# lab-oak/oak

Measured on AMD Instinct MI355X. Metric: turn-steps/s (batched playouts), higher is better.
Workload: dtype u16

## Files before the change

include/oakgpu.h:

```cpp
#ifndef OAKGPU_H
#define OAKGPU_H
#include <stddef.h>
#include <stdint.h>

#ifdef __cplusplus
extern "C" {
#endif

#define OAKGPU_BATTLE_SIZE 384
#define OAKGPU_DURATIONS_SIZE 8
#define OAKGPU_ACTIONS_SIZE 16
#define OAKGPU_MAX_CHOICES 9
#define OAKGPU_TEAMS_SIZE 60

typedef struct oakgpu_ctx oakgpu_ctx;
typedef struct oakgpu_net oakgpu_net;

int oakgpu_create(oakgpu_ctx **out, int device);
void oakgpu_destroy(oakgpu_ctx *ctx);
const char *oakgpu_last_error(void);
int oakgpu_set_stream(oakgpu_ctx *ctx, void *hip_stream);
void *oakgpu_get_stream(oakgpu_ctx *ctx);
int oakgpu_synchronize(oakgpu_ctx *ctx);
int oakgpu_set_kernel_timing(oakgpu_ctx *ctx, int on);
int oakgpu_get_leaf_kernel_ms(oakgpu_ctx *ctx, float ms[3]);
int oakgpu_set_playouts_per_lane(oakgpu_ctx *ctx, int k);
int oakgpu_set_regroup(oakgpu_ctx *ctx, int rounds, int suspend_below, int shrink);
int oakgpu_set_tail_pack(oakgpu_ctx *ctx, int below, int waves, int lanes);
int oakgpu_set_queue_order(oakgpu_ctx *ctx, int on);
int oakgpu_set_spread(oakgpu_ctx *ctx, int lanes);
int oakgpu_set_migration(oakgpu_ctx *ctx, int mode, int long_steps, int adopters);
int oakgpu_set_migration_window(oakgpu_ctx *ctx, int window);
int oakgpu_set_standstill_skip(oakgpu_ctx *ctx, int on);
#define OAKGPU_MOVE_CARRY_DEFAULT 32
int oakgpu_set_move_carry(oakgpu_ctx *ctx, int below);
#define OAKGPU_MOVE_CARRY_DRY_DEFAULT 0
int oakgpu_set_move_carry_dry(oakgpu_ctx *ctx, int below);
#define OAKGPU_LEAN_ROLLOUT_DEFAULT 1
int oakgpu_set_lean_rollout(oakgpu_ctx *ctx, int on);
int oakgpu_last_launch_lean(oakgpu_ctx *ctx);
#define OAKGPU_CTL_FAST_FORWARDED 44
#define OAKGPU_CTL_SKIPPED_STEPS 45
int oakgpu_get_queue_counters(oakgpu_ctx *ctx, uint32_t *out64);
int oakgpu_device_count(void);

int oakgpu_rollout_dev(oakgpu_ctx *ctx, const uint8_t *battles, const uint8_t *durations,
                       const uint8_t *results_in, uint8_t *prng_state, uint32_t n, uint32_t max_steps,
                       int prep, uint8_t *results_out, uint32_t *steps_out, float *values_out,
                       uint8_t *battles_out, uint8_t *durations_out);
int oakgpu_rollout(oakgpu_ctx *ctx, const uint8_t *battles, const uint8_t *durations,
                   const uint8_t *results_in, uint8_t *prng_state, uint32_t n, uint32_t max_steps, int prep,
                   uint8_t *results_out, uint32_t *steps_out, float *values_out, uint8_t *battles_out,
                   uint8_t *durations_out);

typedef struct {
  const uint8_t *battles, *durations, *results_in;
  uint8_t *prng_state;
  uint32_t n;
  uint8_t *results_out;
  uint32_t *steps_out;
  float *values_out;
// ... 619 lines not shown
```

oak_amd/_lib.py:

```python
import ctypes as C
import os

_HERE = os.path.dirname(os.path.abspath(__file__))
LIB_PATH = os.environ.get("OAKGPU_LIB") or os.path.join(_HERE, "liboakgpu.so")

SYMBOLS = [
    "oakgpu_create", "oakgpu_destroy", "oakgpu_last_error", "oakgpu_set_stream", "oakgpu_get_stream", "oakgpu_synchronize", "oakgpu_set_kernel_timing", "oakgpu_get_leaf_kernel_ms", "oakgpu_set_playouts_per_lane", "oakgpu_set_regroup", "oakgpu_set_tail_pack", "oakgpu_set_queue_order", "oakgpu_queue_order", "oakgpu_set_spread", "oakgpu_set_migration", "oakgpu_set_migration_window", "oakgpu_set_standstill_skip", "oakgpu_set_move_carry", "oakgpu_set_move_carry_dry", "oakgpu_set_lean_rollout", "oakgpu_last_launch_lean", "oakgpu_get_queue_counters",
    "oakgpu_device_count", "oakgpu_rollout_dev", "oakgpu_rollout", "oakgpu_rollout_group_dev", "oakgpu_rollout_group",
    "oakgpu_mt19937_fill", "oakgpu_rollout_draws_dev", "oakgpu_rollout_shared_device", "oakgpu_update_dev", "oakgpu_update",
    "oakgpu_choices_dev", "oakgpu_choices", "oakgpu_init_battles_dev", "oakgpu_init_battles",
    "oakgpu_set_ou_pools", "oakgpu_random_ou_battles_dev",
    "oakgpu_net_load", "oakgpu_net_load_memory", "oakgpu_net_free", "oakgpu_net_shape", "oakgpu_net_set_main_precision", "oakgpu_net_main_precision", "oakgpu_net_policy_form",
    "oakgpu_net_load_discrete", "oakgpu_net_load_discrete_memory", "oakgpu_net_is_discrete", "oakgpu_leaf_eval_discrete_raw_dev",
    "oakgpu_leaf_eval_dev", "oakgpu_leaf_eval", "oakgpu_leaf_eval_cached_dev", "oakgpu_leaf_cache_last_count", "oakgpu_leaf_embed_forms", "oakgpu_leaf_eval_policy_dev", "oakgpu_leaf_eval_policy",
    "oakgpu_heap_create", "oakgpu_heap_destroy", "oakgpu_heap_empty", "oakgpu_heap_clear", "oakgpu_heap_kind", "oakgpu_heap_nodes", "oakgpu_heap_update",
    "oakgpu_heap_root_stats", "oakgpu_heap_child_stats", "oakgpu_search_heap", "oakgpu_search_agent_heap", "oakgpu_heap_check_shards", "oakgpu_heap_selftest",
    "oakgpu_tree_step_dev", "oakgpu_search", "oakgpu_search_many", "oakgpu_search_agent", "oakgpu_agent_networks_clear", "oakgpu_bandit_replay", "oakgpu_bandit_select_run", "oakgpu_solve_matrix",
    "oakgpu_segment_mean_dev", "oakgpu_comm_unique_id", "oakgpu_comm_create", "oakgpu_comm_destroy", "oakgpu_all_gather_dev",
    "oakgpu_root_steps_create", "oakgpu_root_steps_destroy", "oakgpu_root_steps_launch_dev", "oakgpu_root_steps_capacity", "oakgpu_root_steps_reserve",
    "oakgpu_endless_battle_check", "oakgpu_frames_size", "oakgpu_frames_write", "oakgpu_frames_read", "oakgpu_selfplay_game", "oakgpu_selfplay_games", "oakgpu_poke_engine_eval_dev", "oakgpu_poke_engine_eval",
    "oakgpu_replay_index", "oakgpu_replay_records_dev", "oakgpu_replay_records", "oakgpu_engine_switches",
    "oakgpu_corpus_create", "oakgpu_corpus_destroy", "oakgpu_corpus_info", "oakgpu_frames_encode_dev", "oakgpu_frames_sample_dev", "oakgpu_encode_battles_dev",
    "oakgpu_frames_encode", "oakgpu_frames_sample",
    "oakgpu_corpus_frame_bases", "oakgpu_corpus_chunks", "oakgpu_corpus_states_dev", "oakgpu_corpus_states", "oakgpu_corpus_inference_dev", "oakgpu_corpus_loss_dev",
    "oakgpu_corpus_inference", "oakgpu_corpus_evaluate",
    "oakgpu_party_table_create", "oakgpu_party_table_destroy", "oakgpu_party_table_fill_dev", "oakgpu_party_table_fill", "oakgpu_leaf_eval_table_dev",
    "oakgpu_leaf_eval_policy_table_dev", "oakgpu_party_table_last_misses", "oakgpu_party_table_rows", "oakgpu_party_table_width", "oakgpu_party_key", "oakgpu_party_variant",
    "oakgpu_set_search_party_table", "oakgpu_search_party_table_stats", "oakgpu_leaf_eval_table", "oakgpu_leaf_eval_policy_table",
    "oakgpu_policy_games_dev", "oakgpu_policy_games", "oakgpu_policy_games_last_stats",
    "oakgpu_forest_create", "oakgpu_forest_destroy", "oakgpu_forest_check", "oakgpu_forest_search_dev", "oakgpu_forest_search", "oakgpu_forest_nodes",
    "oakgpu_forest_last_stats", "oakgpu_search_stream", "oakgpu_agent_params",
    "oakgpu_forest_selfplay_check", "oakgpu_forest_selfplay_dev", "oakgpu_forest_selfplay_records", "oakgpu_forest_selfplay", "oakgpu_forest_selfplay_last_stats",
    "oakgpu_selfplay_pick_host",
    "oakgpu_forest_match_check", "oakgpu_forest_match_dev", "oakgpu_forest_match", "oakgpu_forest_match_last_stats", "oakgpu_match_pick_host",
    "oakgpu_forest_match_set_records", "oakgpu_forest_match_records",
    "oakgpu_forest_create_kept", "oakgpu_forest_create_kept_check", "oakgpu_forest_kept_tree_bytes", "oakgpu_forest_advance_dev", "oakgpu_forest_advance",
    "oakgpu_forest_search_kept_dev", "oakgpu_forest_search_kept", "oakgpu_forest_keep_stats", "oakgpu_forest_mismatch", "oakgpu_forest_node_counts",
    "oakgpu_forest_selfplay_nodes_kept", "oakgpu_forest_selfplay_keep_stats",
    "oakgpu_nash_solve_dev", "oakgpu_solve_matrices", "oakgpu_nash_soft_host", "oakgpu_nash_round_host", "oakgpu_nash_width4_max_entry",
    "oakgpu_forest_selfplay_last_traffic",
# ... 192 lines not shown
    "pkmn_gen1_battle_options_chance_actions", "pkmn_gen1_battle_options_chance_durations",
    "pkmn_result_type", "pkmn_result_p1", "pkmn_result_p2",
]

_lib = None


class OakGpuError(RuntimeError):
    pass


def load():
    global _lib
    if _lib is not None:
        return _lib
    if not os.path.exists(LIB_PATH):
        raise OakGpuError("liboakgpu.so not built: run `python -c 'import __graft_entry__ as g; g.build()'` "
                          "(hipcc --offload-arch=gfx950); there is no CPU fallback")
    lib = C.CDLL(LIB_PATH)
    vp, u32, u64, i32 = C.c_void_p, C.c_uint32, C.c_uint64, C.c_int
    lib.oakgpu_create.argtypes = [C.POINTER(vp), i32]
    lib.oakgpu_destroy.argtypes = [vp]
    lib.oakgpu_destroy.restype = None
    lib.oakgpu_last_error.restype = C.c_char_p
    lib.oakgpu_set_stream.argtypes = [vp, vp]
    lib.oakgpu_get_stream.argtypes = [vp]
    lib.oakgpu_get_stream.restype = vp
    lib.oakgpu_synchronize.argtypes = [vp]
    lib.oakgpu_set_kernel_timing.argtypes = [vp, i32]
    lib.oakgpu_get_leaf_kernel_ms.argtypes = [vp, C.POINTER(C.c_float)]
    lib.oakgpu_set_playouts_per_lane.argtypes = [vp, i32]
    lib.oakgpu_set_regroup.argtypes = [vp, i32, i32, i32]
    lib.oakgpu_set_tail_pack.argtypes = [vp, i32, i32, i32]
    lib.oakgpu_set_queue_order.argtypes = [vp, i32]
    lib.oakgpu_queue_order.argtypes = [vp, C.POINTER(RolloutBatch), u32, vp, C.POINTER(u32)]
    lib.oakgpu_set_spread.argtypes = [vp, i32]
    lib.oakgpu_set_migration.argtypes = [vp, i32, i32, i32]
    lib.oakgpu_set_migration_window.argtypes = [vp, i32]
    lib.oakgpu_set_standstill_skip.argtypes = [vp, i32]
    lib.oakgpu_set_move_carry.argtypes = [vp, i32]
    lib.oakgpu_set_move_carry_dry.argtypes = [vp, i32]
    lib.oakgpu_set_lean_rollout.argtypes = [vp, i32]
    lib.oakgpu_last_launch_lean.argtypes = [vp]
    lib.oakgpu_get_queue_counters.argtypes = [vp, vp]
    lib.oakgpu_rollout_dev.argtypes = [vp, vp, vp, vp, vp, u32, u32, i32, vp, vp, vp, vp, vp]
    lib.oakgpu_rollout.argtypes = [vp, vp, vp, vp, vp, u32, u32, i32, vp, vp, vp, vp, vp]
    lib.oakgpu_rollout_group_dev.argtypes = [vp, C.POINTER(RolloutBatch), u32, u32, i32]
    lib.oakgpu_rollout_group.argtypes = [vp, C.POINTER(RolloutBatch), u32, u32, i32]
    lib.oakgpu_mt19937_fill.argtypes = [u32, u64, vp, C.c_size_t]
    lib.oakgpu_rollout_draws_dev.argtypes = [vp, vp, u32, vp, u32, vp, u32, vp, u32, vp, u32, u32, i32, vp, vp, vp, vp, vp, vp]
    lib.oakgpu_rollout_shared_device.argtypes = [vp, vp, vp, C.c_uint8, vp, u32, u32, u32, i32, vp, vp, vp, vp, vp, vp, vp]
    lib.oakgpu_poke_engine_eval_dev.argtypes = [vp, vp, u32, C.c_float, vp, vp]
    lib.oakgpu_poke_engine_eval.argtypes = [vp, vp, u32, C.c_float, vp, vp]
    lib.oakgpu_tree_step_dev.argtypes = [vp, vp, vp, vp, vp, vp, u32, u32, vp, vp, vp, vp, vp]
    lib.oakgpu_search.argtypes = [vp, vp, vp, vp, C.c_uint8, C.POINTER(SearchParams), C.POINTER(SearchOutput)]
    lib.oakgpu_heap_create.argtypes = [C.POINTER(vp)]
    lib.oakgpu_heap_destroy.argtypes = [vp]
    lib.oakgpu_heap_destroy.restype = None
    lib.oakgpu_heap_empty.argtypes = [vp]
    lib.oakgpu_heap_clear.argtypes = [vp]
    lib.oakgpu_heap_clear.restype = None
    lib.oakgpu_heap_kind.argtypes = [vp]
    lib.oakgpu_heap_nodes.argtypes = [vp]
    lib.oakgpu_heap_nodes.restype = u64
    lib.oakgpu_heap_update.argtypes = [vp, C.c_uint8, C.c_uint8, vp]
    lib.oakgpu_heap_root_stats.argtypes = [vp, i32, vp, vp, vp, vp]
# ... 227 lines not shown
```

oak_amd/csrc/oakgpu.hip:

```cpp
#include <hip/hip_runtime.h>
#include <stdint.h>
#include <stdio.h>
#include <stdlib.h>
#include <string.h>
#include <algorithm>
#include <random>
#include <mutex>
#include <string>
#include <type_traits>
#include <vector>

#include "../../include/oakgpu.h"
#include "gen1_device.hpp"
#include "gen1_regs.hpp"
#include "record_walk.hpp"
#include "oakgpu_internal.h"
#include "fast_prng.hpp"

namespace oak {
using namespace walk;

constexpr int STATE_WORDS = 96;
constexpr int TABLE_LDS_PAD = TABLE_PAD;

// ... 1343 lines not shown
  int device;
  hipStream_t stream;
  bool own_stream;
  uint8_t *d_legal, *d_pools, *d_sizes;
  int n_legal;
  int playouts_per_lane;
  uint32_t *d_queue;
  uint32_t *d_heads;
  int rounds;
  int suspend_below;
  int round_shrink;
  uint8_t *d_scratch;
  size_t scratch_n;
  int rounds_auto;
  int concurrent_hint;
  int search_party_table;
  uint64_t search_table_fills = 0, search_table_evals = 0;
  const void *ws2_owner = nullptr;
  int tail_below;
  int tail_waves;
  int tail_lanes;
  int migrate;
  int migrate_steps;
  int migrate_adopters;
  int migrate_window;
  int migrate_used;
  int spread_lanes;
  int queue_order;
  int standstill_skip;
  int move_carry;
  int move_carry_dry;
  int lean_rollout;
  int last_launch_lean;
  uint32_t *d_order;
  size_t order_n;
  uint32_t order_pair = 0;
  uint32_t ticket_epoch = 0;
  bool tickets_dirty = true;
  int n_cu;
  static constexpr int TABLE_SLOTS = 8;
  void *h_table, *d_table;
  hipEvent_t table_ev[TABLE_SLOTS];
  uint64_t table_next;
  struct Block { void *p; size_t cap; };
  std::vector<Block> stage;
  size_t stage_cursor;
  Block ws[3];
  int timing;
  hipEvent_t tev[4];
  bool tev_valid;
  Block replay_ws{nullptr, 0};
  Block games_ws{nullptr, 0};
  void *attachment = nullptr;
  void (*attachment_dtor)(void *) = nullptr;
};

static thread_local std::string g_err;
static int fail(hipError_t e, const char *what) {
  g_err = std::string(what) + ": " + hipGetErrorString(e);
  return (int)e;
}
static int bad(const char *what) {
  g_err = what;
  return -1;
}
int oakgpu_fail_hip(int e, const char *what) { return fail((hipError_t)e, what); }
int oakgpu_fail_msg(const char *what) { return bad(what); }
int oakgpu_ctx_device(const oakgpu_ctx *c) { return c->device; }
int oakgpu_ctx_enter(oakgpu_ctx *c) {
  hipError_t e = hipSetDevice(c->device);
  return e == hipSuccess ? 0 : fail(e, "hipSetDevice");
}
static void *grow_block(oakgpu_ctx *c, oakgpu_ctx::Block &b, size_t bytes) {
  if (b.cap >= bytes && b.p) return b.p;
  if (b.p) {
    (void)hipStreamSynchronize(c->stream);
    (void)hipFree(b.p);
    b.p = nullptr;
    b.cap = 0;
  }
  const size_t cap = (bytes + (1u << 20) - 1) & ~(size_t)((1u << 20) - 1);
  hipError_t e = hipMalloc(&b.p, cap);
  if (e != hipSuccess) { b.p = nullptr; fail(e, "hipMalloc(context buffer)"); return nullptr; }
  b.cap = cap;
  return b.p;
}
void **oakgpu_ctx_timing_events(oakgpu_ctx *c) { return c->timing && c->tev_valid ? (void **)c->tev : nullptr; }
void *oakgpu_ctx_workspace(oakgpu_ctx *c, int slot, size_t bytes) {
// ... 110 lines not shown
  c->timing = 0;
  c->tev_valid = false;
  c->rounds_auto = 1;
  c->concurrent_hint = 0;
  c->search_party_table = 0;
  if (const char *env = getenv("OAKGPU_PARTY_TABLE")) c->search_party_table = atoi(env) != 0;
  if (const char *env = getenv("OAKGPU_ROUNDS_AUTO")) c->rounds_auto = atoi(env) != 0;
  {
    hipDeviceProp_t prop;
    hipError_t pe = hipGetDeviceProperties(&prop, device);
    if (pe != hipSuccess) { delete c; return fail(pe, "hipGetDeviceProperties"); }
    c->n_cu = prop.multiProcessorCount > 0 ? prop.multiProcessorCount : 256;
  }
  c->rounds = 4;
  c->suspend_below = 32;
  c->round_shrink = 3;
  c->tail_below = 0;
  c->tail_waves = 0;
  if (const char *env = getenv("OAKGPU_TAIL_BELOW")) c->tail_below = atoi(env) < 0 ? 0 : atoi(env) > 64 ? 64 : atoi(env);
  if (const char *env = getenv("OAKGPU_TAIL_WAVES")) c->tail_waves = atoi(env) < 0 ? 0 : atoi(env);
  c->spread_lanes = -1;
  if (const char *env = getenv("OAKGPU_SPREAD_LANES")) c->spread_lanes = atoi(env) < -1 ? -1 : atoi(env) > 64 ? 64 : atoi(env);
  c->queue_order = 1;
  if (const char *env = getenv("OAKGPU_QUEUE_ORDER")) c->queue_order = atoi(env) != 0;
  c->standstill_skip = 1;
  if (const char *env = getenv("OAKGPU_STANDSTILL_SKIP")) c->standstill_skip = atoi(env) != 0;
  c->move_carry = OAKGPU_MOVE_CARRY_DEFAULT;
  if (const char *env = getenv("OAKGPU_MOVE_CARRY")) c->move_carry = atoi(env) < 0 ? 0 : atoi(env) > 64 ? 64 : atoi(env);
  c->move_carry_dry = OAKGPU_MOVE_CARRY_DRY_DEFAULT;
  if (const char *env = getenv("OAKGPU_MOVE_CARRY_DRY")) c->move_carry_dry = atoi(env) < 0 ? 0 : atoi(env) > 64 ? 64 : atoi(env);
  c->lean_rollout = OAKGPU_LEAN_ROLLOUT_DEFAULT;
  if (const char *env = getenv("OAKGPU_LEAN_ROLLOUT")) c->lean_rollout = atoi(env) != 0;
  c->last_launch_lean = 0;
  c->migrate = 1;
  c->migrate_steps = 300;
  c->migrate_adopters = 0;
  c->migrate_window = 48;
  c->migrate_used = 0;
  if (const char *env = getenv("OAKGPU_MIGRATE")) c->migrate = atoi(env) < 0 ? 0 : atoi(env) > 2 ? 2 : atoi(env);
  if (const char *env = getenv("OAKGPU_MIGRATE_STEPS")) c->migrate_steps = atoi(env) < 1 ? 1 : atoi(env);
  if (const char *env = getenv("OAKGPU_MIGRATE_ADOPTERS")) c->migrate_adopters = atoi(env) < 0 ? 0 : atoi(env);
  if (const char *env = getenv("OAKGPU_MIGRATE_WINDOW")) c->migrate_window = atoi(env) < 0 ? 0 : atoi(env) > 255 ? 255 : atoi(env);
  c->d_order = nullptr;
  c->order_n = 0;
  c->tail_lanes = 0;
  if (const char *env = getenv("OAKGPU_TAIL_LANES")) c->tail_lanes = atoi(env) < 0 ? 0 : atoi(env) > 64 ? 64 : atoi(env);
  if (const char *env = getenv("OAKGPU_ROUNDS")) c->rounds = atoi(env) < 1 ? 1 : atoi(env) > 8 ? 8 : atoi(env);
  if (const char *env = getenv("OAKGPU_SUSPEND_BELOW")) c->suspend_below = atoi(env) < 0 ? 0 : atoi(env) > 64 ? 64 : atoi(env);
  if (const char *env = getenv("OAKGPU_ROUND_SHRINK")) c->round_shrink = atoi(env) < 1 ? 1 : atoi(env);
  hipError_t e = hipStreamCreateWithFlags(&c->stream, hipStreamNonBlocking);
  if (e != hipSuccess) { delete c; return fail(e, "hipStreamCreate"); }
  *out = c;
  return 0;
}

void oakgpu_destroy(oakgpu_ctx *c) {
  if (!c) return;
  (void)hipSetDevice(c->device);
  (void)hipStreamSynchronize(c->stream);
  if (c->attachment && c->attachment_dtor) { c->attachment_dtor(c->attachment); c->attachment = nullptr; }
  if (c->own_stream) (void)hipStreamDestroy(c->stream);
  if (c->d_legal) (void)hipFree(c->d_legal);
  if (c->d_pools) (void)hipFree(c->d_pools);
  if (c->d_sizes) (void)hipFree(c->d_sizes);
  if (c->d_queue) (void)hipFree(c->d_queue);
  if (c->d_heads) (void)hipFree(c->d_heads);
  if (c->d_scratch) (void)hipFree(c->d_scratch);
  if (c->d_order) (void)hipFree(c->d_order);
  for (auto &b : c->stage) if (b.p) (void)hipFree(b.p);
  for (auto &b : c->ws) if (b.p) (void)hipFree(b.p);
  if (c->replay_ws.p) (void)hipFree(c->replay_ws.p);
  if (c->games_ws.p) (void)hipFree(c->games_ws.p);
  if (c->tev_valid) for (auto &e : c->tev) (void)hipEventDestroy(e);
  if (c->h_table) {
    (void)hipHostFree(c->h_table);
    (void)hipFree(c->d_table);
    for (int i = 0; i < oakgpu_ctx::TABLE_SLOTS; ++i) (void)hipEventDestroy(c->table_ev[i]);
  }
  delete c;
}

int oakgpu_set_stream(oakgpu_ctx *c, void *hip_stream) {
  if (!c) return bad("null ctx");
  if (c->own_stream) { (void)hipStreamSynchronize(c->stream); (void)hipStreamDestroy(c->stream); }
  c->stream = (hipStream_t)hip_stream;
  c->own_stream = false;
  return 0;
}

int oakgpu_set_playouts_per_lane(oakgpu_ctx *c, int k) {
// ... 65 lines not shown
  return 0;
}

int oakgpu_last_launch_lean(oakgpu_ctx *c) { return c ? c->last_launch_lean : 0; }

int oakgpu_set_search_party_table(oakgpu_ctx *c, int on) {
  if (!c) return bad("null ctx");
  const int old = c->search_party_table;
  c->search_party_table = on != 0;
  return old;
}

int oakgpu_search_party_table_stats(oakgpu_ctx *c, uint64_t *fills, uint64_t *evals) {
  if (!c) return bad("null ctx");
  if (fills) *fills = c->search_table_fills;
  if (evals) *evals = c->search_table_evals;
  return 0;
}

int oakgpu_set_queue_order(oakgpu_ctx *c, int on) {
  if (!c) return bad("null ctx");
  c->queue_order = on != 0;
  return 0;
}

int oakgpu_set_tail_pack(oakgpu_ctx *c, int below, int waves, int lanes) {
  if (!c || below < 0 || below > 64 || waves < 0 || lanes < 0 || lanes > 64) return bad("oakgpu_set_tail_pack: bad argument");
  c->tail_below = below;
  c->tail_waves = waves;
  c->tail_lanes = lanes;
  return 0;
}

void *oakgpu_get_stream(oakgpu_ctx *c) { return c ? (void *)c->stream : nullptr; }

int oakgpu_set_kernel_timing(oakgpu_ctx *c, int on) {
  if (!c) return bad("null ctx");
  HIPCHK(hipSetDevice(c->device));
  if (on && !c->tev_valid) {
    for (auto &e : c->tev) HIPCHK(hipEventCreate(&e));
    c->tev_valid = true;
  }
  c->timing = on != 0;
  return 0;
}

int oakgpu_get_leaf_kernel_ms(oakgpu_ctx *c, float ms[3]) {
  if (!c || !ms) return bad("oakgpu_get_leaf_kernel_ms: null argument");
  if (!c->timing || !c->tev_valid) return bad("oakgpu_get_leaf_kernel_ms: kernel timing is off (oakgpu_set_kernel_timing)");
  HIPCHK(hipEventSynchronize(c->tev[3]));
  for (int i = 0; i < 3; ++i) HIPCHK(hipEventElapsedTime(&ms[i], c->tev[i], c->tev[i + 1]));
  return 0;
}

int oakgpu_synchronize(oakgpu_ctx *c) {
  if (!c) return bad("null ctx");
  HIPCHK(hipStreamSynchronize(c->stream));
  if (c->d_queue && c->migrate_used) {
    uint32_t err = 0;
    HIPCHK(hipMemcpy(&err, c->d_queue + 63, 4, hipMemcpyDeviceToHost));
    c->migrate_used = 0;
    if (err) { HIPCHK(hipMemsetAsync(c->d_queue + 63, 0, 4, c->stream)); HIPCHK(hipStreamSynchronize(c->stream)); }
    if (err) return bad("rollout: a bounded wait of the long-playout migration ran out (playouts were lost) -- oakgpu_set_migration(ctx, 0, ...) turns it off");
  }
  return 0;
}
// ... 27 lines not shown
  const int slot = (int)(c->table_next++ % oakgpu_ctx::TABLE_SLOTS);
  HIPCHK(hipEventSynchronize(c->table_ev[slot]));
  oak::BatchDesc *ht = (oak::BatchDesc *)c->h_table + (size_t)slot * oak::MAX_GROUP, *dt = (oak::BatchDesc *)c->d_table + (size_t)slot * oak::MAX_GROUP;
  memcpy(ht, descs, sizeof(oak::BatchDesc) * count);
  HIPCHK(hipMemcpyAsync(dt, ht, sizeof(oak::BatchDesc) * count, hipMemcpyHostToDevice, c->stream));
  HIPCHK(hipEventRecord(c->table_ev[slot], c->stream));
  *dt_out = dt;
  return 0;
}

static int launch_queue_order(oakgpu_ctx *c, const oak::GroupArgs &g) {
  if (c->order_n < g.total) {
    if (c->d_order) { HIPCHK(hipStreamSynchronize(c->stream)); HIPCHK(hipFree(c->d_order)); c->d_order = nullptr; }
    HIPCHK(hipMalloc((void **)&c->d_order, (size_t)g.total * 4));
    c->order_n = g.total;
  }
  const uint32_t pair = 32u + 2u * c->order_pair;
  c->order_pair ^= 1u;
  hipLaunchKernelGGL(oak::k_queue_order, dim3((g.total + oak::ORDER_PER_BLOCK - 1) / oak::ORDER_PER_BLOCK), dim3(oak::ORDER_BLOCK), 0, c->stream, g, c->d_order,
                     c->d_queue, c->d_heads, pair);
  return 0;
}

static int launch_group(oakgpu_ctx *c, const oak::BatchDesc *descs, uint32_t count, uint32_t total, uint32_t max_steps, int prep) {
  HIPCHK(hipSetDevice(c->device));
  oak::BatchDesc *dt = nullptr;
  if (int r = stage_group_table(c, descs, count, &dt)) return r;
  const uint32_t n64 = (total + 63) / 64;
  uint32_t waves = (n64 + c->playouts_per_lane - 1) / c->playouts_per_lane;
  if (waves < 1) waves = 1;
  const uint32_t resident = (uint32_t)c->n_cu * 4u * 4u;
  bool saturated = waves >= resident;
  if (saturated) waves = resident;
  uint32_t spread = 0;
  if (!saturated && c->spread_lanes != 0 && !c->concurrent_hint && max_steps > 64) {
    const uint64_t slots = ((uint64_t)total + c->playouts_per_lane - 1) / c->playouts_per_lane;
    uint32_t lanes = c->spread_lanes > 0 ? (uint32_t)c->spread_lanes : (uint32_t)((slots + resident - 1) / resident);
    if (lanes < 4) lanes = 4;
    if (lanes < 64) {
      uint32_t w = (uint32_t)((slots + lanes - 1) / lanes);
      if (w > resident) w = resident;
      if (w > waves) { waves = w; spread = lanes; }
    }
  }
  const bool tail_pack = saturated && c->tail_below > 0 && max_steps > 64;
  const uint32_t adopters = (uint32_t)(c->migrate_adopters > 0 ? c->migrate_adopters : (c->n_cu + 3) / 4);
  const bool migrate = !tail_pack && max_steps > (uint32_t)c->migrate_steps && waves > adopters &&
                       (c->migrate == 2 || (c->migrate == 1 && saturated && max_steps >= 500));
  const int rounds = tail_pack ? 2 : migrate ? 1 : ((!c->rounds_auto || (c->concurrent_hint && !saturated && max_steps > 64)) && c->suspend_below > 0 && waves >= 8) ? c->rounds : 1;
  if ((rounds > 1 || migrate) && c->scratch_n < total) {
    if (c->d_scratch) { HIPCHK(hipStreamSynchronize(c->stream)); HIPCHK(hipFree(c->d_scratch)); c->d_scratch = nullptr; }
    HIPCHK(hipMalloc((void **)&c->d_scratch, (size_t)total * (384 + 8 + 4 + 4) + (((size_t)total + 15) & ~(size_t)15)));
    c->scratch_n = total;
    c->tickets_dirty = true;
  }
  const size_t lq = 24 * 64 * 4 + oak::TABLE_LDS_PAD + oak::COLD_LDS_BYTES;
  uint8_t *sb = c->d_scratch, *sd = sb ? sb + (size_t)c->scratch_n * 384 : nullptr;
  uint32_t *lists[2] = {sd ? (uint32_t *)(sd + (size_t)c->scratch_n * 8) : nullptr, nullptr};
  lists[1] = lists[0] ? lists[0] + c->scratch_n : nullptr;
  uint8_t *sres = lists[1] ? (uint8_t *)(lists[1] + c->scratch_n) : nullptr;
  const oak::GroupArgs g{dt, count, total, max_steps, prep};
  bool lean = c->lean_rollout != 0;
  for (uint32_t i = 0; i < count; ++i) lean = lean && !descs[i].durations_out;
  c->last_launch_lean = lean;
  const uint32_t *order = nullptr;
  if (c->queue_order && max_steps > 250 && total >= 8192) {
    if (int r = launch_queue_order(c, g)) return r;
    order = c->d_order;
  } else {
    hipLaunchKernelGGL(oak::k_clear_launch_words, dim3(1), dim3(256), 0, c->stream, c->d_queue, c->d_heads);
  }
  if (migrate) {
    if (++c->ticket_epoch == 0 || c->tickets_dirty) {
      HIPCHK(hipMemsetAsync(lists[0], 0, (size_t)c->scratch_n * 8, c->stream));
      if (c->ticket_epoch == 0) c->ticket_epoch = 1;
      c->tickets_dirty = false;
    }
    c->migrate_used = 1;
  } else if (rounds > 1) c->tickets_dirty = true;
  for (int r = 0; r < rounds; ++r) {
    oak::RoundArgs q{};
    q.order = r == 0 ? order : nullptr;
    q.long_steps = (uint32_t)(c->migrate_steps > 0xFFFF ? 0xFFFF : c->migrate_steps) | (uint32_t)(c->migrate_window > 0 ? c->migrate_window : 256) << 16;
    q.no_skip = c->standstill_skip ? 0u : 1u;
    q.move_carry = (uint32_t)c->move_carry;
    q.stats = c->d_queue + OAKGPU_CTL_FAST_FORWARDED;
    if (migrate) { q.adopt_ctl = c->d_queue + 40; q.adopt_list = (uint64_t *)lists[0]; q.epoch = c->ticket_epoch; q.n_adopters = adopters; }
    q.list_in = r ? lists[(r - 1) & 1] : nullptr;
    q.n_in = r ? c->d_queue + 2 * r - 1 : nullptr;
    q.list_out = lists[r & 1];
    q.count_out = c->d_queue + 2 * r + 1;
    q.sb = sb; q.sd = sd; q.sres = sres;
    q.suspend_below = r + 1 < rounds ? (uint32_t)(tail_pack ? c->tail_below : c->suspend_below) : 0u;
    q.move_carry_dry = c->move_carry_dry > 0 ? std::max((uint32_t)c->move_carry_dry, q.suspend_below) : 0u;
    q.queue = c->d_heads + (size_t)r * oak::QUEUE_HEADS * oak::QUEUE_HEAD_STRIDE;
    q.lanes = (tail_pack && r > 0) ? (uint32_t)c->tail_lanes : (r == 0 ? spread : 0u);
    if (lean && !prep) hipLaunchKernelGGL((oak::k_rollout_queue<64, 4, false, false>), dim3(waves), dim3(64), lq, c->stream, g, q);
    else if (lean) hipLaunchKernelGGL((oak::k_rollout_queue<64, 4, false>), dim3(waves), dim3(64), lq, c->stream, g, q);
    else hipLaunchKernelGGL((oak::k_rollout_queue<64, 4>), dim3(waves), dim3(64), lq, c->stream, g, q);
    waves = tail_pack ? (uint32_t)(c->tail_waves > 0 ? c->tail_waves : c->n_cu) : (waves + c->round_shrink - 1) / c->round_shrink;
    if (waves < 1) waves = 1;
  }
  HIPCHK(hipGetLastError());
  return 0;
}

int oakgpu_queue_order(oakgpu_ctx *c, const oakgpu_rollout_batch *batches, uint32_t count, uint32_t *order_out, uint32_t *suspects_out) {
  if (!c || !batches || !order_out || count == 0 || count > (uint32_t)oak::MAX_GROUP) return bad("oakgpu_queue_order: bad argument");
  HIPCHK(hipSetDevice(c->device));
  uint64_t total = 0;
  for (uint32_t i = 0; i < count; ++i) { if (!batches[i].battles || batches[i].n == 0) return bad("oakgpu_queue_order: empty batch"); total += batches[i].n; }
  if (total >= 0xFFFFFFF0ull) return bad("oakgpu_queue_order: more than 2^32 playouts");
  uint8_t *d_battles = nullptr;
  HIPCHK(hipMalloc((void **)&d_battles, (size_t)total * 384));
  oak::BatchDesc descs[oak::MAX_GROUP] = {};
  uint32_t start = 0;
  int rc = 0;
  for (uint32_t i = 0; i < count && !rc; ++i) {
    descs[i].battles = d_battles + (size_t)start * 384;
    descs[i].start = start;
    descs[i].n = batches[i].n;
    if (hipMemcpyAsync(d_battles + (size_t)start * 384, batches[i].battles, (size_t)batches[i].n * 384, hipMemcpyHostToDevice, c->stream) != hipSuccess) rc = bad("oakgpu_queue_order: copy");
    start += batches[i].n;
  }
  oak::BatchDesc *dt = nullptr;
  if (!rc) rc = stage_group_table(c, descs, count, &dt);
  uint32_t pair = 32u + 2u * c->order_pair;
  if (!rc) rc = launch_queue_order(c, oak::GroupArgs{dt, count, (uint32_t)total, 1000u, 0});
  if (!rc && hipGetLastError() != hipSuccess) rc = bad("oakgpu_queue_order: launch");
  if (!rc && hipMemcpyAsync(order_out, c->d_order, (size_t)total * 4, hipMemcpyDeviceToHost, c->stream) != hipSuccess) rc = bad("oakgpu_queue_order: copy back");
  uint32_t suspects = 0;
  if (!rc && hipMemcpyAsync(&suspects, c->d_queue + pair, 4, hipMemcpyDeviceToHost, c->stream) != hipSuccess) rc = bad("oakgpu_queue_order: copy back");
  hipError_t se = hipStreamSynchronize(c->stream);
// ... 611 lines not shown
```

oak_amd/engine.py:

```python
import ctypes as C
import os

import numpy as np

from . import _lib, gamedata


def _p(a):
    return None if a is None else a.ctypes.data_as(C.c_void_p)


def _u8(a, shape=None):
    a = np.ascontiguousarray(a, dtype=np.uint8)
    return a if shape is None else a.reshape(shape)


class Context:

    def __init__(self, device=0):
        self.lib = _lib.load()
        h = C.c_void_p()
        _lib.check(self.lib.oakgpu_create(C.byref(h), device))
        self.handle = h
        self.device = device
# ... 32 lines not shown

    def set_migration_window(self, window=48):
        _lib.check(self.lib.oakgpu_set_migration_window(self.handle, int(window)))

    def set_search_party_table(self, on=True):
        return bool(self.lib.oakgpu_set_search_party_table(self.handle, int(bool(on))))

    def search_party_table_stats(self):
        fills, evals = C.c_uint64(), C.c_uint64()
        _lib.check(self.lib.oakgpu_search_party_table_stats(self.handle, C.byref(fills), C.byref(evals)))
        return fills.value, evals.value

    def queue_order(self, battles_per_batch):
        bs = [_u8(b) for b in battles_per_batch]
        descs = (_lib.RolloutBatch * len(bs))()
        for k, b in enumerate(bs):
            descs[k].battles, descs[k].n = b.ctypes.data, b.shape[0]
        order = np.zeros(sum(b.shape[0] for b in bs), dtype=np.uint32)
        suspects = C.c_uint32(0)
        _lib.check(self.lib.oakgpu_queue_order(self.handle, descs, len(bs), _p(order), C.byref(suspects)))
        return order, suspects.value

    def set_move_carry(self, below=0):
        _lib.check(self.lib.oakgpu_set_move_carry(self.handle, int(below)))

    def set_move_carry_dry(self, below=0):
        _lib.check(self.lib.oakgpu_set_move_carry_dry(self.handle, int(below)))

    def set_lean_rollout(self, on=True):
        _lib.check(self.lib.oakgpu_set_lean_rollout(self.handle, 1 if on else 0))

    def last_launch_lean(self):
        return bool(self.lib.oakgpu_last_launch_lean(self.handle))

    def set_standstill_skip(self, on=True):
        _lib.check(self.lib.oakgpu_set_standstill_skip(self.handle, 1 if on else 0))

    def queue_counters(self):
        out = np.zeros(64, dtype=np.uint32)
        _lib.check(self.lib.oakgpu_get_queue_counters(self.handle, out.ctypes.data_as(C.c_void_p)))
        return out


    def stream_ptr(self):
        return self.lib.oakgpu_get_stream(self.handle)

    def synchronize(self):
        _lib.check(self.lib.oakgpu_synchronize(self.handle))

    def ensure_ou_pools(self):
        if not self._pools:
            legal, pools, sizes = gamedata.ou_pools()
            _lib.check(self.lib.oakgpu_set_ou_pools(self.handle, _p(legal), len(legal),
                                                    _p(np.ascontiguousarray(pools)), _p(sizes)))
            self._pools = True

    def rollout(self, battles, durations, results, prng, max_steps=1000, prep=False, return_state=False, return_durations=True):
        battles = _u8(battles)
        n = battles.shape[0]
        durations = _u8(durations, (n, 8))
        results = _u8(results, (n,))
        prng = _u8(prng, (n, 8)).copy()
        out = np.zeros(n, dtype=np.uint8)
        steps = np.zeros(n, dtype=np.uint32)
        values = np.zeros(n, dtype=np.float32)
        bo = np.zeros((n, 384), dtype=np.uint8) if return_state else None
# ... 206 lines not shown
```

Baseline: 12.16 billion.

## Add yield schedule that shrinks launches when contexts share a saturated device

Adds a process-wide registry of live contexts. When a saturated long rollout launches while another context on the same device has launched more recently, the launch holds back a slice of its waves and runs as a two-round tail-pack: the first round parks playouts below a threshold and a smaller second round finishes them. The aim is to let concurrent contexts interleave on the GPU instead of each filling every CU, which reduces contention and tail idling. The cost is a mutex on every launch, an extra kernel round, scratch memory, and fewer waves in the first round.

```diff
diff --git a/include/oakgpu.h b/include/oakgpu.h
--- a/include/oakgpu.h
+++ b/include/oakgpu.h
@@ -27,6 +27,14 @@
 int oakgpu_set_playouts_per_lane(oakgpu_ctx *ctx, int k);
 int oakgpu_set_regroup(oakgpu_ctx *ctx, int rounds, int suspend_below, int shrink);
 int oakgpu_set_tail_pack(oakgpu_ctx *ctx, int below, int waves, int lanes);
+#define OAKGPU_YIELD_SCHEDULE_DEFAULT 1
+#define OAKGPU_YIELD_BELOW_DEFAULT 12
+#define OAKGPU_YIELD_WAVES_DEFAULT 256
+#define OAKGPU_YIELD_LANES_DEFAULT 0
+int oakgpu_set_yield_schedule(oakgpu_ctx *ctx, int mode, int below, int waves, int lanes);
+int oakgpu_set_yield_saturation(oakgpu_ctx *ctx, int waves);
+int oakgpu_last_launch_yield(oakgpu_ctx *ctx);
+int oakgpu_last_launch_parked(oakgpu_ctx *ctx, uint32_t *parked);
 int oakgpu_set_queue_order(oakgpu_ctx *ctx, int on);
 int oakgpu_set_spread(oakgpu_ctx *ctx, int lanes);
 int oakgpu_set_migration(oakgpu_ctx *ctx, int mode, int long_steps, int adopters);
diff --git a/oak_amd/_lib.py b/oak_amd/_lib.py
--- a/oak_amd/_lib.py
+++ b/oak_amd/_lib.py
@@ -5,7 +5,7 @@
 LIB_PATH = os.environ.get("OAKGPU_LIB") or os.path.join(_HERE, "liboakgpu.so")
 
 SYMBOLS = [
-    "oakgpu_create", "oakgpu_destroy", "oakgpu_last_error", "oakgpu_set_stream", "oakgpu_get_stream", "oakgpu_synchronize", "oakgpu_set_kernel_timing", "oakgpu_get_leaf_kernel_ms", "oakgpu_set_playouts_per_lane", "oakgpu_set_regroup", "oakgpu_set_tail_pack", "oakgpu_set_queue_order", "oakgpu_queue_order", "oakgpu_set_spread", "oakgpu_set_migration", "oakgpu_set_migration_window", "oakgpu_set_standstill_skip", "oakgpu_set_move_carry", "oakgpu_set_move_carry_dry", "oakgpu_set_lean_rollout", "oakgpu_last_launch_lean", "oakgpu_get_queue_counters",
+    "oakgpu_create", "oakgpu_destroy", "oakgpu_last_error", "oakgpu_set_stream", "oakgpu_get_stream", "oakgpu_synchronize", "oakgpu_set_kernel_timing", "oakgpu_get_leaf_kernel_ms", "oakgpu_set_playouts_per_lane", "oakgpu_set_regroup", "oakgpu_set_tail_pack", "oakgpu_set_yield_schedule", "oakgpu_set_yield_saturation", "oakgpu_last_launch_yield", "oakgpu_last_launch_parked", "oakgpu_set_queue_order", "oakgpu_queue_order", "oakgpu_set_spread", "oakgpu_set_migration", "oakgpu_set_migration_window", "oakgpu_set_standstill_skip", "oakgpu_set_move_carry", "oakgpu_set_move_carry_dry", "oakgpu_set_lean_rollout", "oakgpu_last_launch_lean", "oakgpu_get_queue_counters",
     "oakgpu_device_count", "oakgpu_rollout_dev", "oakgpu_rollout", "oakgpu_rollout_group_dev", "oakgpu_rollout_group",
     "oakgpu_mt19937_fill", "oakgpu_rollout_draws_dev", "oakgpu_rollout_shared_device", "oakgpu_update_dev", "oakgpu_update",
     "oakgpu_choices_dev", "oakgpu_choices", "oakgpu_init_battles_dev", "oakgpu_init_battles",
@@ -264,6 +264,10 @@
     lib.oakgpu_set_playouts_per_lane.argtypes = [vp, i32]
     lib.oakgpu_set_regroup.argtypes = [vp, i32, i32, i32]
     lib.oakgpu_set_tail_pack.argtypes = [vp, i32, i32, i32]
+    lib.oakgpu_set_yield_schedule.argtypes = [vp, i32, i32, i32, i32]
+    lib.oakgpu_set_yield_saturation.argtypes = [vp, i32]
+    lib.oakgpu_last_launch_yield.argtypes = [vp]
+    lib.oakgpu_last_launch_parked.argtypes = [vp, C.POINTER(u32)]
     lib.oakgpu_set_queue_order.argtypes = [vp, i32]
     lib.oakgpu_queue_order.argtypes = [vp, C.POINTER(RolloutBatch), u32, vp, C.POINTER(u32)]
     lib.oakgpu_set_spread.argtypes = [vp, i32]
diff --git a/oak_amd/csrc/oakgpu.hip b/oak_amd/csrc/oakgpu.hip
--- a/oak_amd/csrc/oakgpu.hip
+++ b/oak_amd/csrc/oakgpu.hip
@@ -1399,6 +1399,14 @@
   int move_carry_dry;
   int lean_rollout;
   int last_launch_lean;
+  int yield_mode;
+  int yield_below;
+  int yield_waves;
+  int yield_lanes;
+  int yield_min_waves;
+  uint64_t sat_seq = 0;
+  int last_launch_yield;
+  int last_launch_rounds;
   uint32_t *d_order;
   size_t order_n;
   uint32_t order_pair = 0;
@@ -1421,6 +1429,22 @@
   void *attachment = nullptr;
   void (*attachment_dtor)(void *) = nullptr;
 };
+
+static std::mutex g_yield_mu;
+static std::vector<oakgpu_ctx *> g_live_ctx;
+static uint64_t g_sat_seq = 0;
+static void yield_registry_add(oakgpu_ctx *c) { std::lock_guard<std::mutex> lock(g_yield_mu); g_live_ctx.push_back(c); }
+static void yield_registry_remove(oakgpu_ctx *c) {
+  std::lock_guard<std::mutex> lock(g_yield_mu);
+  for (size_t i = 0; i < g_live_ctx.size(); ++i) if (g_live_ctx[i] == c) { g_live_ctx[i] = g_live_ctx.back(); g_live_ctx.pop_back(); break; }
+}
+static bool yield_registry_launch(oakgpu_ctx *c) {
+  std::lock_guard<std::mutex> lock(g_yield_mu);
+  bool other = false;
+  if (c->sat_seq) for (const oakgpu_ctx *o : g_live_ctx) other |= o != c && o->device == c->device && o->sat_seq > c->sat_seq;
+  c->sat_seq = ++g_sat_seq;
+  return other;
+}
 
 static thread_local std::string g_err;
 static int fail(hipError_t e, const char *what) {
@@ -1597,6 +1621,16 @@
   c->lean_rollout = OAKGPU_LEAN_ROLLOUT_DEFAULT;
   if (const char *env = getenv("OAKGPU_LEAN_ROLLOUT")) c->lean_rollout = atoi(env) != 0;
   c->last_launch_lean = 0;
+  c->yield_mode = OAKGPU_YIELD_SCHEDULE_DEFAULT;
+  c->yield_below = OAKGPU_YIELD_BELOW_DEFAULT;
+  c->yield_waves = OAKGPU_YIELD_WAVES_DEFAULT;
+  c->yield_lanes = OAKGPU_YIELD_LANES_DEFAULT;
+  c->yield_min_waves = 0;
+  c->last_launch_yield = c->last_launch_rounds = 0;
+  if (const char *env = getenv("OAKGPU_YIELD_SCHEDULE")) c->yield_mode = atoi(env) < 0 ? 0 : atoi(env) > 2 ? 2 : atoi(env);
+  if (const char *env = getenv("OAKGPU_YIELD_BELOW")) c->yield_below = atoi(env) < 1 ? 1 : atoi(env) > 64 ? 64 : atoi(env);
+  if (const char *env = getenv("OAKGPU_YIELD_WAVES")) c->yield_waves = atoi(env) < 0 ? 0 : atoi(env);
+  if (const char *env = getenv("OAKGPU_YIELD_LANES")) c->yield_lanes = atoi(env) < 0 ? 0 : atoi(env) > 64 ? 64 : atoi(env);
   c->migrate = 1;
   c->migrate_steps = 300;
   c->migrate_adopters = 0;
@@ -1615,12 +1649,14 @@
   if (const char *env = getenv("OAKGPU_ROUND_SHRINK")) c->round_shrink = atoi(env) < 1 ? 1 : atoi(env);
   hipError_t e = hipStreamCreateWithFlags(&c->stream, hipStreamNonBlocking);
   if (e != hipSuccess) { delete c; return fail(e, "hipStreamCreate"); }
+  yield_registry_add(c);
   *out = c;
   return 0;
 }
 
 void oakgpu_destroy(oakgpu_ctx *c) {
   if (!c) return;
+  yield_registry_remove(c);
   (void)hipSetDevice(c->device);
   (void)hipStreamSynchronize(c->stream);
   if (c->attachment && c->attachment_dtor) { c->attachment_dtor(c->attachment); c->attachment = nullptr; }
@@ -1752,6 +1788,33 @@
   return 0;
 }
 
+int oakgpu_set_yield_schedule(oakgpu_ctx *c, int mode, int below, int waves, int lanes) {
+  if (!c || mode < 0 || mode > 2 || below < 1 || below > 64 || waves < 0 || lanes < 0 || lanes > 64) return bad("oakgpu_set_yield_schedule: bad argument");
+  c->yield_mode = mode;
+  c->yield_below = below;
+  c->yield_waves = waves;
+  c->yield_lanes = lanes;
+  return 0;
+}
+
+int oakgpu_set_yield_saturation(oakgpu_ctx *c, int waves) {
+  if (!c || waves < 0) return bad("oakgpu_set_yield_saturation: bad argument");
+  c->yield_min_waves = waves;
+  return 0;
+}
+
+int oakgpu_last_launch_yield(oakgpu_ctx *c) { return c ? c->last_launch_yield : 0; }
+
+int oakgpu_last_launch_parked(oakgpu_ctx *c, uint32_t *parked) {
+  if (!c || !parked) return bad("oakgpu_last_launch_parked: null argument");
+  *parked = 0;
+  if (!c->d_queue || c->last_launch_rounds < 2) return 0;
+  HIPCHK(hipSetDevice(c->device));
+  HIPCHK(hipMemcpyAsync(parked, c->d_queue + 1, 4, hipMemcpyDeviceToHost, c->stream));
+  HIPCHK(hipStreamSynchronize(c->stream));
+  return 0;
+}
+
 void *oakgpu_get_stream(oakgpu_ctx *c) { return c ? (void *)c->stream : nullptr; }
 
 int oakgpu_set_kernel_timing(oakgpu_ctx *c, int on) {
@@ -1845,8 +1908,21 @@
   const uint32_t resident = (uint32_t)c->n_cu * 4u * 4u;
   bool saturated = waves >= resident;
   if (saturated) waves = resident;
+  bool yield = false;
+  uint32_t yield_r = 0;
+  {
+    const bool ysat = max_steps >= 500 && (saturated || (c->yield_min_waves > 0 && waves >= (uint32_t)c->yield_min_waves));
+    const bool alternating = ysat && yield_registry_launch(c);
+    yield = waves >= 2 && (c->yield_mode == 2 || (c->yield_mode == 1 && alternating));
+    if (yield) {
+      yield_r = (uint32_t)(c->yield_waves > 0 ? c->yield_waves : c->n_cu);
+      if (yield_r * 2 > waves) yield_r = waves / 4 ? waves / 4 : 1;
+      waves -= yield_r;
+    }
+  }
+  c->last_launch_yield = yield;
   uint32_t spread = 0;
-  if (!saturated && c->spread_lanes != 0 && !c->concurrent_hint && max_steps > 64) {
+  if (!yield && !saturated && c->spread_lanes != 0 && !c->concurrent_hint && max_steps > 64) {
     const uint64_t slots = ((uint64_t)total + c->playouts_per_lane - 1) / c->playouts_per_lane;
     uint32_t lanes = c->spread_lanes > 0 ? (uint32_t)c->spread_lanes : (uint32_t)((slots + resident - 1) / resident);
     if (lanes < 4) lanes = 4;
@@ -1856,11 +1932,14 @@
       if (w > waves) { waves = w; spread = lanes; }
     }
   }
-  const bool tail_pack = saturated && c->tail_below > 0 && max_steps > 64;
+  const bool tail_pack = yield || (saturated && c->tail_below > 0 && max_steps > 64);
+  const int tail_below = yield ? c->yield_below : c->tail_below, tail_lanes = yield ? c->yield_lanes : c->tail_lanes;
+  const uint32_t tail_waves = yield ? yield_r : (uint32_t)(c->tail_waves > 0 ? c->tail_waves : c->n_cu);
   const uint32_t adopters = (uint32_t)(c->migrate_adopters > 0 ? c->migrate_adopters : (c->n_cu + 3) / 4);
   const bool migrate = !tail_pack && max_steps > (uint32_t)c->migrate_steps && waves > adopters &&
                        (c->migrate == 2 || (c->migrate == 1 && saturated && max_steps >= 500));
   const int rounds = tail_pack ? 2 : migrate ? 1 : ((!c->rounds_auto || (c->concurrent_hint && !saturated && max_steps > 64)) && c->suspend_below > 0 && waves >= 8) ? c->rounds : 1;
+  c->last_launch_rounds = rounds;
   if ((rounds > 1 || migrate) && c->scratch_n < total) {
     if (c->d_scratch) { HIPCHK(hipStreamSynchronize(c->stream)); HIPCHK(hipFree(c->d_scratch)); c->d_scratch = nullptr; }
     HIPCHK(hipMalloc((void **)&c->d_scratch, (size_t)total * (384 + 8 + 4 + 4) + (((size_t)total + 15) & ~(size_t)15)));
@@ -1904,14 +1983,14 @@
     q.list_out = lists[r & 1];
     q.count_out = c->d_queue + 2 * r + 1;
     q.sb = sb; q.sd = sd; q.sres = sres;
-    q.suspend_below = r + 1 < rounds ? (uint32_t)(tail_pack ? c->tail_below : c->suspend_below) : 0u;
+    q.suspend_below = r + 1 < rounds ? (uint32_t)(tail_pack ? tail_below : c->suspend_below) : 0u;
     q.move_carry_dry = c->move_carry_dry > 0 ? std::max((uint32_t)c->move_carry_dry, q.suspend_below) : 0u;
     q.queue = c->d_heads + (size_t)r * oak::QUEUE_HEADS * oak::QUEUE_HEAD_STRIDE;
-    q.lanes = (tail_pack && r > 0) ? (uint32_t)c->tail_lanes : (r == 0 ? spread : 0u);
+    q.lanes = (tail_pack && r > 0) ? (uint32_t)tail_lanes : (r == 0 ? spread : 0u);
     if (lean && !prep) hipLaunchKernelGGL((oak::k_rollout_queue<64, 4, false, false>), dim3(waves), dim3(64), lq, c->stream, g, q);
     else if (lean) hipLaunchKernelGGL((oak::k_rollout_queue<64, 4, false>), dim3(waves), dim3(64), lq, c->stream, g, q);
     else hipLaunchKernelGGL((oak::k_rollout_queue<64, 4>), dim3(waves), dim3(64), lq, c->stream, g, q);
-    waves = tail_pack ? (uint32_t)(c->tail_waves > 0 ? c->tail_waves : c->n_cu) : (waves + c->round_shrink - 1) / c->round_shrink;
+    waves = tail_pack ? tail_waves : (waves + c->round_shrink - 1) / c->round_shrink;
     if (waves < 1) waves = 1;
   }
   HIPCHK(hipGetLastError());
diff --git a/oak_amd/engine.py b/oak_amd/engine.py
--- a/oak_amd/engine.py
+++ b/oak_amd/engine.py
@@ -88,6 +88,20 @@
 
     def last_launch_lean(self):
         return bool(self.lib.oakgpu_last_launch_lean(self.handle))
+
+    def set_yield_schedule(self, mode=0, below=12, waves=256, lanes=0):
+        _lib.check(self.lib.oakgpu_set_yield_schedule(self.handle, int(mode), int(below), int(waves), int(lanes)))
+
+    def set_yield_saturation(self, waves=0):
+        _lib.check(self.lib.oakgpu_set_yield_saturation(self.handle, int(waves)))
+
+    def last_launch_yield(self):
+        return bool(self.lib.oakgpu_last_launch_yield(self.handle))
+
+    def last_launch_parked(self):
+        n = C.c_uint32(0)
+        _lib.check(self.lib.oakgpu_last_launch_parked(self.handle, C.byref(n)))
+        return n.value
 
     def set_standstill_skip(self, on=True):
         _lib.check(self.lib.oakgpu_set_standstill_skip(self.handle, 1 if on else 0))
```

Result: faster. 12.95 billion (median of 6 runs) (+6.5%).
